# ansonb/RECON

Measured on AMD Instinct MI355X. Metric: edges aggregated/sec (GAT fwd+bwd) on synthetic KG-context graphs, higher is better.
Workload: dtype f32

## Files before the change

recon_amd/csrc/gat_atp.hip:

```cpp
#include <math.h>
#include <stdlib.h>
#include "recon_common.h"

#include <type_traits>

namespace recon {
namespace {

constexpr int kBlock = 256;

__device__ __forceinline__ int xcd_block(int b, int nb) {
    const int q = nb >> 3, r = nb & 7, x = b & 7, i = b >> 3;
    return (x < r ? x * (q + 1) : r * (q + 1) + (x - r) * q) + i;
}
template <int VEC, bool B16>
__device__ __forceinline__ void load_in(float (&r)[VEC], const float* base, int64_t e) {
    if constexpr (!B16) {
        load_vec<VEC>(r, base + e);
    } else {
        const uint16_t* b = reinterpret_cast<const uint16_t*>(base) + e;
        if constexpr (VEC == 4) {
            const uint2 t = *reinterpret_cast<const uint2*>(b);
            r[0] = __builtin_bit_cast(float, t.x << 16); r[1] = __builtin_bit_cast(float, t.x & 0xffff0000u);
            r[2] = __builtin_bit_cast(float, t.y << 16); r[3] = __builtin_bit_cast(float, t.y & 0xffff0000u);
// ... 1305 lines not shown
#endif
        if (hv && writer) {
            if (is_piece) p.hubG[static_cast<int64_t>(widx) * H + myh] = sum_gs;
            else p.Gs_dst[static_cast<int64_t>(node) * 2 * H + myh] = sum_gs;
        }
#pragma unroll
        for (int h = 0; h < HT; ++h) {
            if (h0 + h < H) {
                const float sh = lane_bcast(sum_gs, h << SH);
                const float* uh = U + (h0 + h) * UW;
#pragma unroll
                for (int r = 0; r < KR; ++r) {
                    float ud[VEC];
                    load_vec<VEC>(ud, uh + uF[r]);
#pragma unroll
                    for (int v = 0; v < VEC; ++v) gxd[r][v] = fmaf(sh, ud[v], gxd[r][v]);
                }
            }
        }
    }
    if (is_piece) return;
#ifdef RECON_K2_STAMPS
    stamp_[4] = __builtin_readcyclecounter();
    stamp_[5] = __builtin_amdgcn_s_getreg((31 << 11) | 4);
    if (lane == 0) {
        uint64_t* o = reinterpret_cast<uint64_t*>(p.gxd + static_cast<int64_t>(node) * F);
        for (int i = 0; i < 6; ++i) o[i] = stamp_[i];
        o[6] = static_cast<uint64_t>(end - beg);
    }
    if (!more) return;
    node = nnode; beg = nbeg; end = nend; srcv0 = nidx[0]; eidv0 = nidx[64];
    stamp_[0] = __builtin_readcyclecounter();
    continue;
#endif
    const auto rgx = K2_RSRC(p.gxd + static_cast<int64_t>(node) * F, F * 4);
#pragma unroll
    for (int r = 0; r < KR; ++r) buf_store_f32<VEC>(gxd[r], rgx, voF[r]);
    if (!more) return;
    node = nnode; beg = nbeg; end = nend; srcv0 = nidx[0]; eidv0 = nidx[64];
    }
}

template <int VEC>
__global__ void __launch_bounds__(kBlock) k_gat_atp_hub_bwd(const AtpBwdK p, const int32_t* __restrict__ hub_node, const int32_t* __restrict__ hub_ptr,
                                                            int32_t n_hub) {
    const int lane = threadIdx.x & 63;
    const int wave = __builtin_amdgcn_readfirstlane(threadIdx.x >> 6);
    const int t = blockIdx.x * (kBlock / 64) + wave;
    const int F = p.F, R = p.R, H = p.H, W = 2 * F + R;
    if (t >= n_hub) return;
    const int node = hub_node[t], p0 = hub_ptr[t], p1 = hub_ptr[t + 1];
    float tot = 0.f;
    if (lane < H) {
        float tt[1] = {0.f};
        sum_pieces<1>(tt, p.hubG + lane, H, p0, p1);
        tot = tt[0];
        p.Gs_dst[static_cast<int64_t>(node) * 2 * H + lane] += tot;
    }
    for (int c = lane * VEC; c < F; c += 64 * VEC) {
        float o[VEC];
        load_vec<VEC>(o, p.gxd + static_cast<int64_t>(node) * F + c);
        for (int h = 0; h < H; ++h) {
            const float sh = lane_bcast(tot, h);
            float ud[VEC];
            load_vec<VEC>(ud, p.u + static_cast<int64_t>(h) * W + c);
#pragma unroll
            for (int v = 0; v < VEC; ++v) o[v] = fmaf(sh, ud[v], o[v]);
        }
        store_vec<VEC>(p.gxd + static_cast<int64_t>(node) * F + c, o);
    }
}

struct AtpSrcK {
    const int32_t* rowptr_src; const int32_t* slot_by_src; const float* Gxs; const float* gxd; const float* gsigma;
    float* g_x; float* Gs_src;
    const float* u; int32_t W;
    int32_t N, F, H;
    int32_t hub_chunk, n_piece;
    const int4* piece;
    float* hubP;
    const int32_t* node_row;
};
template <int VEC, int KR>
__global__ void __launch_bounds__(kBlock) k_gat_atp_src(const AtpSrcK p) {
    const int lane = threadIdx.x & 63;
    const int wave = __builtin_amdgcn_readfirstlane(threadIdx.x >> 6);
    const int npb = (p.n_piece + kBlock / 64 - 1) / (kBlock / 64);
    const int widx = blockIdx.x * (kBlock / 64) + wave;
    const bool is_piece = static_cast<int>(blockIdx.x) < npb;
    int node = xcd_block(blockIdx.x - npb, gridDim.x - npb) * (kBlock / 64) + wave;
    int beg, end;
    if (is_piece) {
        if (widx >= p.n_piece) return;
        const int4 pc = p.piece[widx]; node = pc.x; beg = pc.y; end = pc.z;
    } else {
        if (node >= p.N) return;
        beg = p.rowptr_src[node]; end = p.rowptr_src[node + 1];
        if (p.hub_chunk && end - beg > p.hub_chunk) return;
    }
    const int F = p.F, H = p.H;
    const int drow = (p.node_row && !is_piece) ? p.node_row[node] : node;
    float acc[KR][VEC];
#pragma unroll
    for (int r = 0; r < KR; ++r) {
#pragma unroll
        for (int v = 0; v < VEC; ++v) acc[r][v] = 0.f;
        const int c = (r * 64 + lane) * VEC;
        if (!is_piece && c < F && p.g_x && drow >= 0) load_vec<VEC>(acc[r], p.gxd + static_cast<int64_t>(drow) * F + c);
    }
    float gs = 0.f;
    constexpr int U = 4;
    const int hl = lane < H ? lane : 0;
    for (int c0 = beg; c0 < end; c0 += 64) {
        const int cn = min(64, end - c0);
        const int slotv = p.slot_by_src[c0 + min(lane, cn - 1)];
        for (int j0 = 0; j0 < cn; j0 += U) {
            int slot[U];
#pragma unroll
            for (int u = 0; u < U; ++u) slot[u] = __builtin_amdgcn_readlane(slotv, min(j0 + u, cn - 1));
            float g4[U], t[U][KR][VEC];
#pragma unroll
            for (int u = 0; u < U; ++u) {
                g4[u] = p.gsigma[static_cast<int64_t>(slot[u]) * H + hl];
                if (p.g_x) {
#pragma unroll
                    for (int r = 0; r < KR; ++r) {
                        const int c = (r * 64 + lane) * VEC;
                        load_vec<VEC>(t[u][r], p.Gxs + static_cast<int64_t>(slot[u]) * F + (c < F ? c : 0));
                    }
                }
            }
#pragma unroll
            for (int u = 0; u < U; ++u) {
                if (j0 + u < cn) {
                    gs += g4[u];
                    if (p.g_x) {
#pragma unroll
                        for (int r = 0; r < KR; ++r)
#pragma unroll
                            for (int v = 0; v < VEC; ++v) acc[r][v] += t[u][r][v];
                    }
                }
            }
        }
    }
    float* gs_out = is_piece ? p.hubP + static_cast<int64_t>(widx) * (F + H) + F : p.Gs_src + static_cast<int64_t>(node) * 2 * H + H;
    float* row_out = is_piece ? p.hubP + static_cast<int64_t>(widx) * (F + H) : p.g_x + static_cast<int64_t>(node) * F;
    if (lane < H) gs_out[lane] = gs;
    if (!is_piece && p.g_x) {
        constexpr int HBK = KR <= 2 ? 8 : 2;
        for (int hb = 0; hb < H; hb += HBK) {
            float us[HBK][KR][VEC];
#pragma unroll
            for (int t = 0; t < HBK; ++t) {
                const float* uh = p.u + static_cast<int64_t>(min(hb + t, H - 1)) * p.W + F;
#pragma unroll
                for (int r = 0; r < KR; ++r) {
                    const int c = (r * 64 + lane) * VEC;
                    load_vec<VEC>(us[t][r], uh + (c < F ? c : 0));
                }
            }
#pragma unroll
            for (int t = 0; t < HBK; ++t) {
                const float sh = hb + t < H ? lane_bcast(gs, min(hb + t, 63)) : 0.f;
#pragma unroll
                for (int r = 0; r < KR; ++r)
#pragma unroll
                    for (int v = 0; v < VEC; ++v) acc[r][v] = fmaf(sh, us[t][r][v], acc[r][v]);
            }
        }
    }
    if (p.g_x) {
#pragma unroll
        for (int r = 0; r < KR; ++r) {
            const int c = (r * 64 + lane) * VEC;
            if (c < F) {
                if (is_piece && ((F + H) % VEC)) {
#pragma unroll
                    for (int v = 0; v < VEC; ++v) row_out[c + v] = acc[r][v];
                } else store_vec<VEC>(row_out + c, acc[r]);
            }
        }
    }
}

__global__ void __launch_bounds__(kBlock) k_gat_atp_hub_src(const AtpSrcK p, const int32_t* __restrict__ hub_node, const int32_t* __restrict__ hub_ptr,
                                                            int32_t n_hub) {
    const int lane = threadIdx.x & 63;
    const int F = p.F, H = p.H;
    const int stripes = (F + 63) / 64;
    const int idx = blockIdx.x * (kBlock / 64) + __builtin_amdgcn_readfirstlane(threadIdx.x >> 6);
    if (idx >= n_hub * stripes) return;
    const int t = idx / stripes, c = (idx - t * stripes) * 64 + lane;
    const int node = hub_node[t], p0 = hub_ptr[t], p1 = hub_ptr[t + 1];
    float gsl[1] = {0.f};
    if (lane < H) sum_pieces<1>(gsl, p.hubP + F + lane, F + H, p0, p1);
    if (c < H) p.Gs_src[static_cast<int64_t>(node) * 2 * H + H + c] = gsl[0];
    if (!p.g_x) return;
    const int drow = p.node_row ? p.node_row[node] : node;
    float a[1] = {(c < F && drow >= 0) ? p.gxd[static_cast<int64_t>(drow) * F + c] : 0.f};
    if (c < F) sum_pieces<1>(a, p.hubP + c, F + H, p0, p1);
    for (int h = 0; h < H; ++h) a[0] = fmaf(lane_bcast(gsl[0], h), p.u[static_cast<int64_t>(h) * p.W + F + (c < F ? c : 0)], a[0]);
    if (c < F) p.g_x[static_cast<int64_t>(node) * F + c] = a[0];
}


struct SkinnyJob { const float* G; const float* X; const int32_t* gather; float* partial; int32_t ldg, nj, rows, K, rpb, nb; };
template <int NJ, bool B16 = false>
__global__ void __launch_bounds__(256) k_skinny_tn_partial(const SkinnyJob j0, const SkinnyJob j1, const SkinnyJob j2) {
    __shared__ float red[3][NJ][256];
    const int which = static_cast<int>(blockIdx.x) < j0.nb ? 0 : (static_cast<int>(blockIdx.x) < j0.nb + j1.nb ? 1 : 2);
    const SkinnyJob& jb = which == 0 ? j0 : (which == 1 ? j1 : j2);
    const float* __restrict__ G = jb.G;
    const float* __restrict__ X = jb.X;
    const int32_t* __restrict__ gather = jb.gather;
    float* __restrict__ partial = jb.partial;
    const int ldg = jb.ldg, nj = jb.nj, rows = jb.rows, K = jb.K, rows_per_block = jb.rpb;
    const int bid = blockIdx.x - (which == 0 ? 0 : (which == 1 ? j0.nb : j0.nb + j1.nb));
    const int lane = threadIdx.x & 63, wave = threadIdx.x >> 6;
    const int r0 = bid * rows_per_block;
    const int r1 = min(rows, r0 + rows_per_block);
    for (int c0 = 0; c0 < K; c0 += 256) {
        const int c = c0 + 4 * lane;
        float acc[NJ][4];
#pragma unroll
        for (int j = 0; j < NJ; ++j) acc[j][0] = acc[j][1] = acc[j][2] = acc[j][3] = 0.f;
        int gi = 0;
        if (gather && lane < 4 && r0 + wave * 4 + lane < r1) gi = gather[r0 + wave * 4 + lane];
        for (int rb = r0 + wave * 4; rb < r1; rb += 16) {
            int gnext = 0;
            if (gather && lane < 4 && rb + 16 + lane < r1) gnext = gather[rb + 16 + lane];
            float xv[4][4];
            float gl = 0.f;
            {
                const int q = lane / NJ, j = lane % NJ;
                if (q < 4 && rb + q < r1 && j < nj) gl = G[static_cast<int64_t>(rb + q) * ldg + j];
            }
#pragma unroll
            for (int q = 0; q < 4; ++q) {
                const int r = rb + q;
                xv[q][0] = xv[q][1] = xv[q][2] = xv[q][3] = 0.f;
                if (r < r1) {
                    const int64_t row = gather ? __builtin_amdgcn_readlane(gi, q) : r;
                    if constexpr (B16) {
                        if (c + 3 < K) load_in<4, true>(xv[q], X, row * K + c);
                    } else {
                        if (c + 3 < K) { const float4 t = *reinterpret_cast<const float4*>(X + row * K + c); xv[q][0] = t.x; xv[q][1] = t.y; xv[q][2] = t.z; xv[q][3] = t.w; }
                        else { for (int v = 0; v < 4; ++v) if (c + v < K) xv[q][v] = X[row * K + c + v]; }
                    }
                }
            }
            gi = gnext;
            float gv[4][NJ];
#pragma unroll
            for (int q = 0; q < 4; ++q)
#pragma unroll
                for (int j = 0; j < NJ; ++j) gv[q][j] = (q * NJ + j < 64) ? lane_bcast(gl, (q * NJ + j) & 63) : 0.f;
#pragma unroll
            for (int q = 0; q < 4; ++q)
#pragma unroll
                for (int j = 0; j < NJ; ++j)
#pragma unroll
                    for (int v = 0; v < 4; ++v) acc[j][v] = fmaf(gv[q][j], xv[q][v], acc[j][v]);
        }
        __syncthreads();
        if (wave > 0) {
#pragma unroll
            for (int j = 0; j < NJ; ++j)
#pragma unroll
                for (int v = 0; v < 4; ++v) red[wave - 1][j][4 * lane + v] = acc[j][v];
        }
        __syncthreads();
        if (wave == 0) {
#pragma unroll
            for (int j = 0; j < NJ; ++j)
                if (j < nj)
#pragma unroll
                    for (int v = 0; v < 4; ++v)
                        if (c + v < K)
                            partial[(static_cast<int64_t>(bid) * nj + j) * K + c + v] =
                                ((acc[j][v] + red[0][j][4 * lane + v]) + red[1][j][4 * lane + v]) + red[2][j][4 * lane + v];
        }
    }
}
struct SkinnyRedJob { const float* partial; float* out; int64_t S1, S2; int32_t nb, nj, K, P, nblocks; };
__global__ void __launch_bounds__(1024) k_skinny_reduce(const SkinnyRedJob j0, const SkinnyRedJob j1, const SkinnyRedJob j2) {
    __shared__ float red[64][17];
    const int which = static_cast<int>(blockIdx.x) < j0.nblocks ? 0 : (static_cast<int>(blockIdx.x) < j0.nblocks + j1.nblocks ? 1 : 2);
    const SkinnyRedJob& jb = which == 0 ? j0 : (which == 1 ? j1 : j2);
    const float* __restrict__ partial = jb.partial;
    float* __restrict__ out = jb.out;
    const int nb = jb.nb, nj = jb.nj, K = jb.K, P = jb.P;
    const int64_t S1 = jb.S1, S2 = jb.S2;
    const int bid = blockIdx.x - (which == 0 ? 0 : (which == 1 ? j0.nblocks : j0.nblocks + j1.nblocks));
    const int e = threadIdx.x & 15, grp = threadIdx.x >> 4;
    const int idx = bid * 16 + e;
    const int tot = nj * K;
    const int per = (nb + 63) / 64;
    const int b0 = grp * per, b1 = min(nb, (grp + 1) * per);
    float s0 = 0.f, s1 = 0.f, s2 = 0.f, s3 = 0.f;
    if (idx < tot) {
        int b = b0;
        for (; b + 4 <= b1; b += 4) {
            s0 += partial[static_cast<int64_t>(b) * tot + idx];
            s1 += partial[static_cast<int64_t>(b + 1) * tot + idx];
            s2 += partial[static_cast<int64_t>(b + 2) * tot + idx];
            s3 += partial[static_cast<int64_t>(b + 3) * tot + idx];
        }
        for (; b < b1; ++b) s0 += partial[static_cast<int64_t>(b) * tot + idx];
    }
    red[grp][e] = (s0 + s1) + (s2 + s3);
    __syncthreads();
    if (grp == 0 && idx < tot) {
        float t = 0.f;
#pragma unroll
        for (int g = 0; g < 64; ++g) t += red[g][e];
        const int j = idx / K, c = idx % K;
        out[(j % P) * S1 + (j / P) * S2 + c] = t;
    }
}

struct AtpShape { int vec, kr, ht; };
bool atp_shape(int F, int R, int H, AtpShape* s) {
    const int mx = F > R ? F : R;
    int vec;
    if (F % 4 == 0 && R % 4 == 0) vec = 4;
    else if (F % 2 == 0 && R % 2 == 0) vec = 2;
    else return false;
    int kr = (mx + 64 * vec - 1) / (64 * vec);
    if (kr > 2 && kr <= 4) kr = 4; else if (kr > 4 && kr <= 8) kr = 8; else if (kr > 8) return false;
    int ht = 1;
    while (ht < H && ht < 8) ht <<= 1;
    while (ht > 1 && 2 * ht * kr * vec > 96) ht >>= 1;
    if (2 * ht * kr * vec > 96) return false;
    s->vec = vec; s->kr = kr; s->ht = ht;
    return true;
}
bool al(const void* p, size_t a) { return (reinterpret_cast<uintptr_t>(p) & (a - 1)) == 0; }
int atp_key(const AtpShape& s) { return s.vec * 1000 + s.kr * 10 + (s.ht == 8 ? 3 : s.ht == 4 ? 2 : s.ht == 2 ? 1 : 0); }

#define ATP_DISPATCH(S, CALL)                                                                              \
    do {                                                                                                   \
        const int key_ = atp_key(S);                                                                       \
        switch (key_) {                                                                                    \
            case 4010: CALL(4, 1, 1); break; case 4011: CALL(4, 1, 2); break; case 4012: CALL(4, 1, 4); break; case 4013: CALL(4, 1, 8); break; \
            case 4020: CALL(4, 2, 1); break; case 4021: CALL(4, 2, 2); break; case 4022: CALL(4, 2, 4); break;   \
            case 4040: CALL(4, 4, 1); break; case 4041: CALL(4, 4, 2); break; case 4080: CALL(4, 8, 1); break;   \
            case 2010: CALL(2, 1, 1); break; case 2011: CALL(2, 1, 2); break; case 2012: CALL(2, 1, 4); break; case 2013: CALL(2, 1, 8); break; \
            case 2020: CALL(2, 2, 1); break; case 2021: CALL(2, 2, 2); break; case 2022: CALL(2, 2, 4); break; case 2023: CALL(2, 2, 8); break; \
            case 2040: CALL(2, 4, 1); break; case 2041: CALL(2, 4, 2); break; case 2042: CALL(2, 4, 4); break;   \
            case 2080: CALL(2, 8, 1); break; case 2081: CALL(2, 8, 2); break;                                   \
            default: return RECON_ERR_UNSUPPORTED;                                                         \
        }                                                                                                  \
    } while (0)

int check_atp(const recon_graph* g, const recon_gat_atp_args* a) {
    if (!g || !a) return RECON_ERR_INVALID;
    if (a->N != g->N || a->E != g->E) return RECON_ERR_INVALID;
    if (a->N < 0 || a->E < 0 || a->F <= 0 || a->R <= 0 || a->D <= 0 || a->H <= 0) return RECON_ERR_INVALID;
    if (a->ld_out < a->H * a->D) return RECON_ERR_INVALID;
    if (!a->x || !a->a || !a->a_2 || !a->u || !a->c_node || !a->V || !a->out) return RECON_ERR_INVALID;
    if (a->E > 0 && (!a->edge_embed || !a->c_rel)) return RECON_ERR_INVALID;
    if (a->H > 4096) return RECON_ERR_UNSUPPORTED;
    if (a->ee_index && a->E > 0 && a->ee_rows <= 0) return RECON_ERR_INVALID;
    return RECON_OK;
}

// ... 211 lines not shown

extern "C" int recon_gat_atp_project(const recon_graph* g, const recon_gat_atp_args* a, recon_stream_t stream) {
    AtpShape s;
    int rc = atp_fwd_common(g, a, &s);
    if (rc != RECON_OK) return rc;
    if (a->N == 0) return RECON_OK;
    const int32_t W = 2 * a->F + a->R;
    const int32_t NR = atp_rows(g, a).n;
    OperandDesc A = plain_operand(a->V, static_cast<int64_t>(a->H) * W);
    OperandDesc B = plain_operand(a->a, W);
    OutputDesc C = plain_output(a->out, a->ld_out);
    GemmBatch bt;
    bt.batch = a->H; bt.a_bs = W; bt.b_bs = static_cast<int64_t>(a->D) * W; bt.c_bs = a->D;
    bt.epilogue = a->concat ? 1 : 0;
    if (atp_hx2(a))
        return gemm_hx2_batched(NR, a->D, W, a->V, W, 2LL * W, 2LL * NR * W, a->a_split, C, bt, atp_scale_v(a), atp_scale_a(a),
                                as_stream(stream), atp_dst_shared(a));
    if (a->a_split && bx3_supported(A, W, bt)) return gemm_bx3_batched(NR, a->D, W, A, a->a_split, C, bt, as_stream(stream));
    return gemm_f32_batched(NR, a->D, W, A, true, B, true, C, bt, 1, nullptr, as_stream(stream));
}

namespace {
__global__ void __launch_bounds__(kBlock) k_rows_expand(const float* __restrict__ rows, int32_t ld_rows, const int32_t* __restrict__ node_row, int32_t N,
                                                        int32_t width, float* __restrict__ out, int32_t ld_out, int32_t vec4) {
    const int lane = threadIdx.x & 63;
    const int n = blockIdx.x * (kBlock / 64) + __builtin_amdgcn_readfirstlane(threadIdx.x >> 6);
    if (n >= N) return;
    const int r = node_row[n];
    float* o = out + static_cast<int64_t>(n) * ld_out;
    const float* in = rows + static_cast<int64_t>(r < 0 ? 0 : r) * ld_rows;
    if (vec4) {
        for (int c = 4 * lane; c < width; c += 256) {
            const float4 v = r >= 0 ? *reinterpret_cast<const float4*>(in + c) : make_float4(0.f, 0.f, 0.f, 0.f);
            *reinterpret_cast<float4*>(o + c) = v;
        }
    } else {
        for (int c = lane; c < width; c += 64) o[c] = r >= 0 ? in[c] : 0.f;
    }
}
}
extern "C" int recon_rows_expand(const float* rows, int32_t ld_rows, const int32_t* node_row, int32_t N, int32_t width, float* out, int32_t ld_out,
                                 recon_stream_t stream) {
    if (N < 0 || width < 0 || ld_rows < width || ld_out < width || (N > 0 && (!node_row || !out)) || (N > 0 && width > 0 && !rows)) return RECON_ERR_INVALID;
    if (N == 0 || width == 0) return RECON_OK;
    const int vec4 = ((width | ld_rows | ld_out) & 3) == 0 && !((reinterpret_cast<uintptr_t>(rows) | reinterpret_cast<uintptr_t>(out)) & 15);
    hipLaunchKernelGGL(k_rows_expand, dim3(static_cast<unsigned>(ceil_div64(N, kBlock / 64))), dim3(kBlock), 0, as_stream(stream), rows, ld_rows, node_row, N, width, out,
                       ld_out, vec4);
    RECON_CHECK_LAUNCH();
    return RECON_OK;
}

extern "C" int recon_gat_atp_fwd(const recon_graph* g, const recon_gat_atp_args* a, recon_stream_t stream) {
    int rc = recon_gat_atp_scores(g, a, stream);
    if (rc != RECON_OK) return rc;
    rc = recon_gat_atp_aggregate(g, a, stream);
    if (rc != RECON_OK) return rc;
    return recon_gat_atp_project(g, a, stream);
}

extern "C" int recon_gat_atp_bwd_gee_bf16_supported(int32_t F, int32_t R, int32_t D, int32_t H) {
    recon::AtpShape s;
    if (!recon_gat_atp_bf16_io_supported(F, R, D, H) || !recon::atp_shape(F, R, H, &s)) return 0;
    const size_t lds_k2 = static_cast<size_t>(H) * (F + R) * sizeof(float) + (kBlock / 64) * 512;
    const bool lring = s.vec == 4 && s.kr == 1 && lds_k2 + (kBlock / 64) * kK2LdsRingBytes <= 64 * 1024 && cfg_char(CFG_K2_LDS_RING) != '0';
    return (s.ht >= H && lring) ? 1 : 0;
}

extern "C" size_t recon_gat_atp_bwd_split_bytes(int32_t N, int32_t D, int32_t H) {
    if (N <= 0 || D <= 0 || H <= 0) return 256;
    return align_up(static_cast<size_t>(3) * N * bx3_kp(H * D) * 2, 256);
}

extern "C" size_t recon_gat_atp_bwd_partial_floats(int32_t N, int32_t E, int32_t F, int32_t R, int32_t D, int32_t H) {
    const int64_t W = 2LL * F + R;
    int s1 = gemm_pick_split_k(static_cast<int32_t>(W), D, N, H);
    const int s2 = bx3_kmajor_splits(N, bx3_kmajor_split_k(static_cast<int32_t>(W), D, N, H));
    if (s2 > s1) s1 = s2;
    size_t need = static_cast<size_t>(s1) * H * D * W;
    (void)E; (void)F; (void)R;
    return need > 0 ? need : 1;
}

constexpr int kSkinnySlices = 1024;
extern "C" size_t recon_gat_atp_bwd_partial2_floats(int32_t N, int32_t E, int32_t F, int32_t R, int32_t D, int32_t H) {
    (void)N; (void)E; (void)D; (void)H;
    const size_t mx = static_cast<size_t>(F > R ? F : R);
    return static_cast<size_t>(3) * kSkinnySlices * 16 * mx;
}

extern "C" int recon_gat_atp_bwd(const recon_graph* g, const recon_gat_atp_bwd_args* b, recon_stream_t stream) {
    return recon_gat_atp_bwd_phase(g, b, RECON_ATP_BWD_ALL, stream);
}

extern "C" int recon_gat_atp_bwd_phase(const recon_graph* g, const recon_gat_atp_bwd_args* b, int32_t phases, recon_stream_t stream) {
    if (!b) return RECON_ERR_INVALID;
    const recon_gat_atp_args* a = &b->fwd;
    int rc = check_atp(g, a);
    if (rc != RECON_OK) return rc;
    if (!recon_gat_atp_supported(a->N, a->E, a->F, a->R, a->D, a->H)) return RECON_ERR_UNSUPPORTED;
    if (!a->Z || !a->Zk || !b->grad_out || !b->g_V || !b->gxd || !b->Gs || !b->g_u || !b->partial || !b->partial2 || !b->q) return RECON_ERR_INVALID;
    if (a->E > 0 && (!a->sigma || !b->g_sigma || !b->Gxs)) return RECON_ERR_INVALID;
    const bool hx2 = atp_hx2(a);
    if ((a->concat || atp_rows(g, a).row_node) && !b->g_h && !hx2) return RECON_ERR_INVALID;
    if (hx2 && (!b->gh_split || (reinterpret_cast<uintptr_t>(b->gh_split) & 15) || (b->ld_gout & 3))) return RECON_ERR_INVALID;
    if (b->ld_gout < a->H * a->D) return RECON_ERR_INVALID;
    if (a->N == 0) return RECON_OK;
    hipStream_t st = as_stream(stream);
    const int32_t N = a->N, E = a->E, F = a->F, R = a->R, D = a->D, H = a->H, W = 2 * F + R;
    const AtpRows rw = atp_rows(g, a);
    const int32_t NR = rw.n;
    const int64_t HD = 1LL * H * D;
    AtpShape s;
    atp_shape(F, R, H, &s);
    const size_t lds_u = static_cast<size_t>(H) * (F + R) * sizeof(float);
    if (lds_u > 60 * 1024) return RECON_ERR_UNSUPPORTED;
    const size_t lds_k2 = lds_u + (kBlock / 64) * 512;

    const float* gh = b->grad_out;
    int32_t ld_gh = b->ld_gout;
    const int64_t ld_ghp = bx3_kp(static_cast<int32_t>(HD));
    const bool gh_planes = hx2 || (b->gh_split && a->a_split && !(reinterpret_cast<uintptr_t>(b->gh_split) & 15) && (D % 8) == 0 &&
                                   ((b->ld_gout | a->ld_out) & 3) == 0);
    uint16_t* ghp = gh_planes ? static_cast<uint16_t*>(b->gh_split) : nullptr;
    const int64_t ldi = (static_cast<int64_t>(NR) + 7) / 8 * 8;
    const size_t inv_off = align_up(static_cast<size_t>(2) * N * bx3_kp(static_cast<int32_t>(HD)) * 2, 256);
    const bool row_scaled = hx2 && D <= 256 && ((a->ld_out | b->ld_gout) & 3) == 0 && cfg_char(CFG_ATP_ROW_SCALE) != '0' &&
                            inv_off + static_cast<size_t>(H) * ldi * sizeof(float) <= recon_gat_atp_bwd_split_bytes(N, D, H);
    float* row_inv = row_scaled ? reinterpret_cast<float*>(static_cast<char*>(b->gh_split) + inv_off) : nullptr;
    if (phases & RECON_ATP_BWD_PREPARE) {
        if (hx2 && !row_scaled) {
            rc = hx2_amax(b->grad_out, N, static_cast<int32_t>(HD), b->ld_gout, atp_q(a, 3), st);
            if (rc != RECON_OK) return rc;
        }
        hipLaunchKernelGGL(k_elu_grad_q, dim3(static_cast<unsigned>(ceil_div64(1LL * NR * H, 16))), dim3(256), 0, st, b->grad_out, b->ld_gout, a->out,
                           a->ld_out, NR, H, D, a->concat, ((a->concat || rw.row_node) && !hx2) ? b->g_h : nullptr, b->q, ghp, hx2 ? 2LL * D : ld_ghp,
                           hx2 ? static_cast<int64_t>(D) : static_cast<int64_t>(NR) * ld_ghp, hx2 ? 1 : 0,
                           hx2 ? atp_scale_g(a) : Hx2Scale{nullptr, nullptr, 1.f}, row_inv, ldi, row_scaled ? atp_q(a, 3) : nullptr, rw.row_node);
    }
    if (a->concat || rw.row_node) { gh = b->g_h; ld_gh = static_cast<int32_t>(HD); }
    GemmBatch bt;
    bt.batch = H; bt.epilogue = 0;
    if (phases & RECON_ATP_BWD_INPUTS) {
    {
        OperandDesc A = plain_operand(gh, ld_gh);
        OperandDesc B = plain_operand(a->a, W);
        OutputDesc C = plain_output(b->g_V, static_cast<int64_t>(H) * W);
        bt.a_bs = D; bt.b_bs = static_cast<int64_t>(D) * W; bt.c_bs = W;
        if (hx2)
            rc = gemm_hx2_batched(NR, W, D, b->gh_split, D, 2LL * D, 2LL * NR * D,
                                  static_cast<const char*>(a->a_split) + split_part_bytes(D, W, H), C, bt,
                                  row_scaled ? Hx2Scale{nullptr, nullptr, 1.f} : atp_scale_g(a), atp_scale_a(a), st, 0, row_inv, ldi);
        else if (a->a_split && bx3_supported(A, D, bt))
            rc = gemm_bx3_batched(NR, W, D, A, static_cast<const char*>(a->a_split) + split_part_bytes(D, W, H), C, bt, st);
        else
            rc = gemm_f32_batched(NR, W, D, A, true, B, false, C, bt, 1, nullptr, st);
        if (rc != RECON_OK) return rc;
    }
    {
        AtpBwdK p;
        p.rowptr = rw.rowptr; p.row_node = rw.row_node; p.src = g->src; p.eid = a->ee_index ? a->ee_index : g->eid;
        p.gee_by_slot = a->ee_index ? 1 : 0;
        p.gee_b16 = b->g_ee_bf16 ? 1 : 0;
        if (b->g_ee_bf16 && !(a->io_bf16 && !a->ee_index && b->g_edge_embed && recon_gat_atp_bwd_gee_bf16_supported(F, R, D, H))) return RECON_ERR_UNSUPPORTED;
        p.x = a->x; p.ee = a->edge_embed; p.keep = a->keep; p.sigma = a->sigma; p.Z = a->Z; p.Zk = a->Zk;
        p.q = b->q; p.gV = b->g_V; p.u = a->u;
        p.gsigma = b->g_sigma; p.Gs_dst = b->Gs; p.Gxs = b->Gxs; p.gxd = b->gxd; p.g_ee = b->g_edge_embed;
        p.N = NR; p.E = E; p.F = F; p.R = R; p.H = H; p.alpha = a->alpha;
        const bool hubs = atp_hubs(g);
        if (hubs && static_cast<size_t>(g->hub_ws_floats) < recon_graph_hub_ws_floats(g, F, R, H)) return RECON_ERR_WORKSPACE;
        p.hub_chunk = hubs ? g->hub_chunk : 0; p.n_piece = hubs ? g->n_piece : 0;
        p.piece = reinterpret_cast<const int4*>(g->piece); p.hubG = g->hub_ws;
        dim3 grid;
        const bool lring = s.vec == 4 && s.kr == 1 && lds_k2 + (kBlock / 64) * kK2LdsRingBytes <= 64 * 1024 && cfg_char(CFG_K2_LDS_RING) != '0';
        const size_t lds_run = lds_k2 + (lring ? (kBlock / 64) * kK2LdsRingBytes : 0);
#define CALL_BWD(V_, K_, H_) do { constexpr bool LRC = V_ == 4 && K_ == 1;                                                                   \
                                  if (V_ == 4 && a->io_bf16) { if (LRC && lring && p.gee_b16) hipLaunchKernelGGL((k_gat_atp_bwd<4, K_, H_, true, LRC, LRC>), grid, dim3(kBlock), lds_run, st, p); \
                                                               else if (LRC && lring) hipLaunchKernelGGL((k_gat_atp_bwd<4, K_, H_, true, LRC>), grid, dim3(kBlock), lds_run, st, p); \
                                                               else hipLaunchKernelGGL((k_gat_atp_bwd<4, K_, H_, true>), grid, dim3(kBlock), lds_run, st, p); }          \
                                  else if (LRC && lring) hipLaunchKernelGGL((k_gat_atp_bwd<V_, K_, H_, false, LRC>), grid, dim3(kBlock), lds_run, st, p);              \
                                  else hipLaunchKernelGGL((k_gat_atp_bwd<V_, K_, H_>), grid, dim3(kBlock), lds_run, st, p); } while (0)
        p.persist = (p.n_piece == 0 && cfg_char(CFG_K2_PERSIST) != '0') ? 1 : 0;
        if (p.persist) {
            const int64_t need = ceil_div64(NR, kBlock / 64);
            int64_t nb = k2_resident_blocks(s.kr, s.ht, lds_run);
            if (nb > need) nb = (need + 7) / 8 * 8;
            grid = dim3(static_cast<unsigned>(nb));
        } else {
            grid = dim3(static_cast<unsigned>(ceil_div64(NR, kBlock / 64) + ceil_div64(p.n_piece, kBlock / 64)));
        }
        ATP_DISPATCH(s, CALL_BWD);
#undef CALL_BWD
        if (hubs) {
            const dim3 gh(static_cast<unsigned>(ceil_div64(g->n_hub, kBlock / 64)));
            if (s.vec == 4) hipLaunchKernelGGL((k_gat_atp_hub_bwd<4>), gh, dim3(kBlock), 0, st, p, g->hub_node, g->hub_ptr, g->n_hub);
            else hipLaunchKernelGGL((k_gat_atp_hub_bwd<2>), gh, dim3(kBlock), 0, st, p, g->hub_node, g->hub_ptr, g->n_hub);
        }
        RECON_CHECK_LAUNCH();
    }
    {
        AtpSrcK p;
        p.rowptr_src = g->rowptr_src; p.slot_by_src = g->slot_by_src; p.Gxs = b->Gxs; p.gxd = b->gxd; p.gsigma = b->g_sigma;
        p.g_x = b->g_x; p.Gs_src = b->Gs; p.u = a->u; p.W = W;
        p.N = N; p.F = F; p.H = H; p.node_row = rw.node_row;
        const bool hubs = g->hub_chunk > 0 && g->n_hub_src > 0 && g->n_piece_src > 0 && g->hub_node_src && g->hub_ptr_src && g->piece_src && g->hub_ws;
        if (hubs && static_cast<size_t>(g->hub_ws_floats) < recon_graph_hub_ws_floats(g, F, R, H)) return RECON_ERR_WORKSPACE;
        p.hub_chunk = hubs ? g->hub_chunk : 0; p.n_piece = hubs ? g->n_piece_src : 0;
        p.piece = reinterpret_cast<const int4*>(g->piece_src); p.hubP = g->hub_ws;
        dim3 grid(static_cast<unsigned>(ceil_div64(N, kBlock / 64) + ceil_div64(p.n_piece, kBlock / 64)));
        const int key = s.vec * 10 + s.kr;
        switch (key) {
            case 41: hipLaunchKernelGGL((k_gat_atp_src<4, 1>), grid, dim3(kBlock), 0, st, p); break;
            case 42: hipLaunchKernelGGL((k_gat_atp_src<4, 2>), grid, dim3(kBlock), 0, st, p); break;
            case 44: hipLaunchKernelGGL((k_gat_atp_src<4, 4>), grid, dim3(kBlock), 0, st, p); break;
            case 48: hipLaunchKernelGGL((k_gat_atp_src<4, 8>), grid, dim3(kBlock), 0, st, p); break;
            case 21: hipLaunchKernelGGL((k_gat_atp_src<2, 1>), grid, dim3(kBlock), 0, st, p); break;
            case 22: hipLaunchKernelGGL((k_gat_atp_src<2, 2>), grid, dim3(kBlock), 0, st, p); break;
            case 24: hipLaunchKernelGGL((k_gat_atp_src<2, 4>), grid, dim3(kBlock), 0, st, p); break;
            default: hipLaunchKernelGGL((k_gat_atp_src<2, 8>), grid, dim3(kBlock), 0, st, p); break;
        }
        if (hubs) hipLaunchKernelGGL(k_gat_atp_hub_src, dim3(static_cast<unsigned>(ceil_div64(1LL * g->n_hub_src * ceil_div64(F, 64), kBlock / 64))), dim3(kBlock), 0, st, p,
                                     g->hub_node_src, g->hub_ptr_src, g->n_hub_src);
        RECON_CHECK_LAUNCH();
    }
    }
    if (b->g_a || b->g_a_2) {
        if (!b->g_a) return RECON_ERR_INVALID;
        if (phases & RECON_ATP_BWD_WEIGHTS) {
            OperandDesc A = plain_operand(a->V, static_cast<int64_t>(H) * W);
            OperandDesc B = plain_operand(gh, ld_gh);
            OutputDesc C = plain_output(b->g_a, W);
            GemmBatch bw = bt;
            bw.a_bs = W; bw.b_bs = D; bw.c_bs = static_cast<int64_t>(D) * W; bw.c_transpose = 1;
            const int64_t ldv = static_cast<int64_t>(H) * W;
            if (hx2) {
                const int sk = bx3_kmajor_splits(NR, bx3_kmajor_split_k(W, D, NR, H));
                rc = gemm_hx2_kmajor_batched(W, D, NR, a->V, 2LL * W, W, 2LL * NR * W, b->gh_split, 2LL * D, D, 2LL * NR * D,
                                             H, sk, b->partial, static_cast<const char*>(a->aux) + kHx2ZeroPageOffset, atp_scale_v(a), atp_scale_g(a), st,
                                             atp_dst_shared(a), row_inv, ldi);
                if (rc == RECON_OK && (phases & RECON_ATP_BWD_EARLY_SUM)) rc = splitk_reduce(b->partial, sk, W, D, C, bw.c_bs, H, 0, true, st);
            } else if (gh_planes && bx3_kmajor_supported(a->V, ldv, W, ld_ghp, D, W, D)) {
                const int sk = bx3_kmajor_splits(NR, bx3_kmajor_split_k(W, D, NR, H));
                rc = gemm_bx3_kmajor_batched(W, D, NR, a->V, ldv, W, b->gh_split, ld_ghp, static_cast<int64_t>(NR) * ld_ghp, D, H, sk, b->partial, st);
                if (rc == RECON_OK) rc = splitk_reduce(b->partial, sk, W, D, C, bw.c_bs, H, 0, true, st);
            } else {
                const int sk = gemm_pick_split_k(W, D, NR, H);
                rc = gemm_f32_batched(W, D, NR, A, false, B, false, C, bw, sk, b->partial, st);
            }
            if (rc != RECON_OK) return rc;
        }
        if (phases & RECON_ATP_BWD_INPUTS) {
            struct Prod { const float* G; int ldg, nj; const float* X; const int32_t* gather; int rows, K, P; int64_t S1, S2; float* out; };
            const int32_t* ee_gather = a->ee_index ? a->ee_index : g->eid;
            const size_t third = recon_gat_atp_bwd_partial2_floats(N, E, F, R, D, H) / 3;
            auto run_jobs = [&](const Prod* pr, int count) {
                SkinnyJob sj[3];
                SkinnyRedJob rj[3];
                int nj_max = 0, nb_total = 0, nr_total = 0;
                for (int i = 0; i < 3; ++i) {
                    sj[i] = SkinnyJob{nullptr, nullptr, nullptr, nullptr, 0, 0, 0, 0, 1, 0};
                    rj[i] = SkinnyRedJob{nullptr, nullptr, 0, 0, 0, 0, 0, 1, 0};
                    if (i >= count) continue;
                    const Prod& q = pr[i];
                    if (q.rows <= 0) {
                        for (int j = 0; j < q.nj; ++j) (void)hipMemsetAsync(q.out + (j % q.P) * q.S1 + (j / q.P) * q.S2, 0, sizeof(float) * q.K, st);
                        continue;
                    }
                    int rpb = static_cast<int>(ceil_div64(q.rows, kSkinnySlices));
                    if (rpb < 32) rpb = 32;
                    const int nb = static_cast<int>(ceil_div64(q.rows, rpb));
                    float* part = b->partial2 + i * third;
                    sj[i] = SkinnyJob{q.G, q.X, q.gather, part, q.ldg, q.nj, q.rows, q.K, rpb, nb};
                    rj[i] = SkinnyRedJob{part, q.out, q.S1, q.S2, nb, q.nj, q.K, q.P, static_cast<int32_t>(ceil_div64(1LL * q.nj * q.K, 16))};
                    if (q.nj > nj_max) nj_max = q.nj;
                    nb_total += nb; nr_total += rj[i].nblocks;
                }
                if (nb_total == 0) return;
                const dim3 gp(static_cast<unsigned>(nb_total));
                if (a->io_bf16) {
                    if (nj_max <= 8) hipLaunchKernelGGL((k_skinny_tn_partial<8, true>), gp, dim3(256), 0, st, sj[0], sj[1], sj[2]);
                    else hipLaunchKernelGGL((k_skinny_tn_partial<16, true>), gp, dim3(256), 0, st, sj[0], sj[1], sj[2]);
                } else if (nj_max <= 8) hipLaunchKernelGGL((k_skinny_tn_partial<8>), gp, dim3(256), 0, st, sj[0], sj[1], sj[2]);
                else hipLaunchKernelGGL((k_skinny_tn_partial<16>), gp, dim3(256), 0, st, sj[0], sj[1], sj[2]);
                hipLaunchKernelGGL(k_skinny_reduce, dim3(static_cast<unsigned>(nr_total)), dim3(1024), 0, st, rj[0], rj[1], rj[2]);
            };
            if (H <= 8) {
                const Prod pr[3] = {{b->Gs, 2 * H, H, a->x, rw.row_node, NR, F, H, W, 0, b->g_u},
                                    {b->Gs + H, 2 * H, H, a->x, nullptr, N, F, H, W, 0, b->g_u + F},
                                    {b->g_sigma, H, H, a->edge_embed, ee_gather, E, R, H, W, 0, b->g_u + 2 * F}};
                run_jobs(pr, 3);
            } else {
                for (int j = 0; j < 2 * H; ++j) {
                    const Prod one = {b->Gs + j, 2 * H, 1, a->x, j < H ? rw.row_node : nullptr, j < H ? NR : N, F, 1, W, 0,
                                      b->g_u + static_cast<int64_t>(j % H) * W + (j / H) * F};
                    run_jobs(&one, 1);
                }
                for (int h0 = 0; h0 < H; h0 += 16) {
                    const int nh = H - h0 < 16 ? H - h0 : 16;
                    const Prod one = {b->g_sigma + h0, H, nh, a->edge_embed, ee_gather, E, R, nh, W, 0, b->g_u + static_cast<int64_t>(h0) * W + 2 * F};
                    run_jobs(&one, 1);
                }
            }
            RECON_CHECK_LAUNCH();
        }
        if ((phases & RECON_ATP_BWD_FINISH) && hx2 && !(phases & RECON_ATP_BWD_EARLY_SUM)) {
            const int sk = bx3_kmajor_splits(NR, bx3_kmajor_split_k(W, D, NR, H));
            const int ntile = static_cast<int>(ceil_div64(W, 32) * ceil_div64(D, 32)) * H;
            hipLaunchKernelGGL(k_atp_weights_finish, dim3(static_cast<unsigned>(ntile + ceil_div64(1LL * H * D, 8))), dim3(256), 0, st, b->partial, sk, W,
                               D, H, a->a, a->a_2, b->g_u, b->g_a, b->g_a_2, atp_q(a, 3), kHx2QuantityWords);
        } else if (phases & RECON_ATP_BWD_FINISH)
        hipLaunchKernelGGL(k_score_vec_bwd, dim3(static_cast<unsigned>(D), static_cast<unsigned>(H)), dim3(256), 0, st, a->a, a->a_2, b->g_u,
                           D, W, b->g_a, b->g_a_2, atp_hx2(a) ? atp_q(a, 3) : nullptr, kHx2QuantityWords);
        RECON_CHECK_LAUNCH();
    } else if ((phases & RECON_ATP_BWD_FINISH) && atp_hx2(a)) {
        if (hipMemsetAsync(atp_q(a, 3), 0, sizeof(uint32_t) * kHx2QuantityWords, st) != hipSuccess) return RECON_ERR_LAUNCH;
    }
    return RECON_OK;
}
```

Measured before the change: 80.92 million.

## Fuse source-gradient kernel with skinny weight-gradient partials in one launch

Merges the per-source-node gradient kernel and the skinny TN weight-gradient partial kernel into a single grid. The first blocks run the source-side wave work and the rest run skinny partial tiles. For the source job, the skinny blocks recompute per-row summed g_sigma from the CSR into LDS instead of reading the Gs source half from global memory, which removes a dependency and lets both kernels overlap. It also cuts the shared reduction buffer from three slices to one, reducing sequentially wave by wave. That lowers LDS use at the cost of extra barriers. The weight-gradient launch moves from the later phase block into the source phase, which may change phase semantics.

```diff
diff --git a/recon_amd/csrc/gat_atp.hip b/recon_amd/csrc/gat_atp.hip
--- a/recon_amd/csrc/gat_atp.hip
+++ b/recon_amd/csrc/gat_atp.hip
@@ -1411,13 +1411,13 @@
     const int32_t* node_row;
 };
 template <int VEC, int KR>
-__global__ void __launch_bounds__(kBlock) k_gat_atp_src(const AtpSrcK p) {
+__device__ __forceinline__ void atp_src_wave(const AtpSrcK& p, int bx, int nbx) {
     const int lane = threadIdx.x & 63;
     const int wave = __builtin_amdgcn_readfirstlane(threadIdx.x >> 6);
     const int npb = (p.n_piece + kBlock / 64 - 1) / (kBlock / 64);
-    const int widx = blockIdx.x * (kBlock / 64) + wave;
-    const bool is_piece = static_cast<int>(blockIdx.x) < npb;
-    int node = xcd_block(blockIdx.x - npb, gridDim.x - npb) * (kBlock / 64) + wave;
+    const int widx = bx * (kBlock / 64) + wave;
+    const bool is_piece = bx < npb;
+    int node = xcd_block(bx - npb, nbx - npb) * (kBlock / 64) + wave;
     int beg, end;
     if (is_piece) {
         if (widx >= p.n_piece) return;
@@ -1512,6 +1512,9 @@
         }
     }
 }
+
+template <int VEC, int KR>
+__global__ void __launch_bounds__(kBlock) k_gat_atp_src(const AtpSrcK p) { atp_src_wave<VEC, KR>(p, blockIdx.x, gridDim.x); }
 
 __global__ void __launch_bounds__(kBlock) k_gat_atp_hub_src(const AtpSrcK p, const int32_t* __restrict__ hub_node, const int32_t* __restrict__ hub_ptr,
                                                             int32_t n_hub) {
@@ -1535,38 +1538,53 @@
 
 
 struct SkinnyJob { const float* G; const float* X; const int32_t* gather; float* partial; int32_t ldg, nj, rows, K, rpb, nb; };
-template <int NJ, bool B16 = false>
-__global__ void __launch_bounds__(256) k_skinny_tn_partial(const SkinnyJob j0, const SkinnyJob j1, const SkinnyJob j2) {
-    __shared__ float red[3][NJ][256];
-    const int which = static_cast<int>(blockIdx.x) < j0.nb ? 0 : (static_cast<int>(blockIdx.x) < j0.nb + j1.nb ? 1 : 2);
-    const SkinnyJob& jb = which == 0 ? j0 : (which == 1 ? j1 : j2);
+struct SkinnySrc { const int32_t* rowptr_src; const int32_t* slot_by_src; const float* gsigma; };
+template <int NJ, bool B16, bool SRC>
+__device__ __forceinline__ void skinny_block(const SkinnyJob& jb, int bid, float (&red)[NJ][256], float* __restrict__ gsl, const SkinnySrc& sr, bool src) {
+    constexpr int RPI = 4;
     const float* __restrict__ G = jb.G;
     const float* __restrict__ X = jb.X;
     const int32_t* __restrict__ gather = jb.gather;
     float* __restrict__ partial = jb.partial;
     const int ldg = jb.ldg, nj = jb.nj, rows = jb.rows, K = jb.K, rows_per_block = jb.rpb;
-    const int bid = blockIdx.x - (which == 0 ? 0 : (which == 1 ? j0.nb : j0.nb + j1.nb));
     const int lane = threadIdx.x & 63, wave = threadIdx.x >> 6;
     const int r0 = bid * rows_per_block;
     const int r1 = min(rows, r0 + rows_per_block);
+    if (SRC && src) {
+        const int n = (r1 - r0) * nj;
+        for (int i = threadIdx.x; i < n; i += 256) {
+            const int rr = i / nj, h = i - rr * nj;
+            const int beg = sr.rowptr_src[r0 + rr], end = sr.rowptr_src[r0 + rr + 1];
+            float gs = 0.f;
+            for (int c0 = beg; c0 < end; c0 += 4) {
+                float g4[4];
+#pragma unroll
+                for (int u = 0; u < 4; ++u) g4[u] = sr.gsigma[static_cast<int64_t>(sr.slot_by_src[min(c0 + u, end - 1)]) * nj + h];
+#pragma unroll
+                for (int u = 0; u < 4; ++u) if (c0 + u < end) gs += g4[u];
+            }
+            gsl[i] = gs;
+        }
+        __syncthreads();
+    }
     for (int c0 = 0; c0 < K; c0 += 256) {
         const int c = c0 + 4 * lane;
         float acc[NJ][4];
 #pragma unroll
         for (int j = 0; j < NJ; ++j) acc[j][0] = acc[j][1] = acc[j][2] = acc[j][3] = 0.f;
         int gi = 0;
-        if (gather && lane < 4 && r0 + wave * 4 + lane < r1) gi = gather[r0 + wave * 4 + lane];
-        for (int rb = r0 + wave * 4; rb < r1; rb += 16) {
+        if (gather && lane < RPI && r0 + wave * RPI + lane < r1) gi = gather[r0 + wave * RPI + lane];
+        for (int rb = r0 + wave * RPI; rb < r1; rb += 4 * RPI) {
             int gnext = 0;
-            if (gather && lane < 4 && rb + 16 + lane < r1) gnext = gather[rb + 16 + lane];
-            float xv[4][4];
+            if (gather && lane < RPI && rb + 4 * RPI + lane < r1) gnext = gather[rb + 4 * RPI + lane];
+            float xv[RPI][4];
             float gl = 0.f;
             {
                 const int q = lane / NJ, j = lane % NJ;
-                if (q < 4 && rb + q < r1 && j < nj) gl = G[static_cast<int64_t>(rb + q) * ldg + j];
-            }
-#pragma unroll
-            for (int q = 0; q < 4; ++q) {
+                if (q < RPI && rb + q < r1 && j < nj) gl = (SRC && src) ? gsl[(rb + q - r0) * nj + j] : G[static_cast<int64_t>(rb + q) * ldg + j];
+            }
+#pragma unroll
+            for (int q = 0; q < RPI; ++q) {
                 const int r = rb + q;
                 xv[q][0] = xv[q][1] = xv[q][2] = xv[q][3] = 0.f;
                 if (r < r1) {
@@ -1580,38 +1598,63 @@
                 }
             }
             gi = gnext;
-            float gv[4][NJ];
-#pragma unroll
-            for (int q = 0; q < 4; ++q)
-#pragma unroll
-                for (int j = 0; j < NJ; ++j) gv[q][j] = (q * NJ + j < 64) ? lane_bcast(gl, (q * NJ + j) & 63) : 0.f;
-#pragma unroll
-            for (int q = 0; q < 4; ++q)
+#pragma unroll
+            for (int q = 0; q < RPI; ++q)
+#pragma unroll
+                for (int j = 0; j < NJ; ++j) {
+                    const float gv = lane_bcast(gl, q * NJ + j);
+#pragma unroll
+                    for (int v = 0; v < 4; ++v) acc[j][v] = fmaf(gv, xv[q][v], acc[j][v]);
+                }
+        }
+        for (int w = 1; w < 4; ++w) {
+            __syncthreads();
+            if (wave == w) {
 #pragma unroll
                 for (int j = 0; j < NJ; ++j)
 #pragma unroll
-                    for (int v = 0; v < 4; ++v) acc[j][v] = fmaf(gv[q][j], xv[q][v], acc[j][v]);
-        }
-        __syncthreads();
-        if (wave > 0) {
-#pragma unroll
-            for (int j = 0; j < NJ; ++j)
-#pragma unroll
-                for (int v = 0; v < 4; ++v) red[wave - 1][j][4 * lane + v] = acc[j][v];
-        }
-        __syncthreads();
+                    for (int v = 0; v < 4; ++v) red[j][4 * lane + v] = acc[j][v];
+            }
+            __syncthreads();
+            if (wave == 0) {
+#pragma unroll
+                for (int j = 0; j < NJ; ++j)
+#pragma unroll
+                    for (int v = 0; v < 4; ++v) acc[j][v] += red[j][4 * lane + v];
+            }
+        }
         if (wave == 0) {
 #pragma unroll
             for (int j = 0; j < NJ; ++j)
                 if (j < nj)
 #pragma unroll
                     for (int v = 0; v < 4; ++v)
-                        if (c + v < K)
-                            partial[(static_cast<int64_t>(bid) * nj + j) * K + c + v] =
-                                ((acc[j][v] + red[0][j][4 * lane + v]) + red[1][j][4 * lane + v]) + red[2][j][4 * lane + v];
-        }
-    }
-}
+                        if (c + v < K) partial[(static_cast<int64_t>(bid) * nj + j) * K + c + v] = acc[j][v];
+        }
+    }
+}
+template <int NJ, bool B16 = false>
+__global__ void __launch_bounds__(256) k_skinny_tn_partial(const SkinnyJob j0, const SkinnyJob j1, const SkinnyJob j2) {
+    __shared__ float red[NJ][256];
+    const int which = static_cast<int>(blockIdx.x) < j0.nb ? 0 : (static_cast<int>(blockIdx.x) < j0.nb + j1.nb ? 1 : 2);
+    const SkinnyJob& jb = which == 0 ? j0 : (which == 1 ? j1 : j2);
+    skinny_block<NJ, B16, false>(jb, blockIdx.x - (which == 0 ? 0 : (which == 1 ? j0.nb : j0.nb + j1.nb)), red, nullptr, SkinnySrc{nullptr, nullptr, nullptr}, false);
+}
+
+template <int VEC, int KR, bool B16>
+__global__ void __launch_bounds__(kBlock) k_gat_atp_src_skinny(const AtpSrcK p, int32_t nsrc, const SkinnyJob j0, const SkinnyJob j1, const SkinnyJob j2,
+                                                               const SkinnySrc sr) {
+    static_assert(kBlock == 256, "skinny_block: 4 waves");
+    __shared__ float red[8][256];
+    extern __shared__ __attribute__((aligned(16))) float gsl[];
+    const int bx = blockIdx.x;
+    if (bx < nsrc) { atp_src_wave<VEC, KR>(p, bx, nsrc); return; }
+    const int b = bx - nsrc;
+    const int which = b < j0.nb ? 0 : (b < j0.nb + j1.nb ? 1 : 2);
+    const SkinnyJob& jb = which == 0 ? j0 : (which == 1 ? j1 : j2);
+    skinny_block<8, B16, true>(jb, b - (which == 0 ? 0 : (which == 1 ? j0.nb : j0.nb + j1.nb)), red, gsl, sr, which == 1);
+}
+
 struct SkinnyRedJob { const float* partial; float* out; int64_t S1, S2; int32_t nb, nj, K, P, nblocks; };
 __global__ void __launch_bounds__(1024) k_skinny_reduce(const SkinnyRedJob j0, const SkinnyRedJob j1, const SkinnyRedJob j2) {
     __shared__ float red[64][17];
@@ -1989,6 +2032,11 @@
 }
 
 constexpr int kSkinnySlices = 1024;
+constexpr size_t kSkinnySrcLdsMax = 32 * 1024;
+static int skinny_rpb(int64_t rows) {
+    const int rpb = static_cast<int>(ceil_div64(rows, kSkinnySlices));
+    return rpb < 32 ? 32 : rpb;
+}
 extern "C" size_t recon_gat_atp_bwd_partial2_floats(int32_t N, int32_t E, int32_t F, int32_t R, int32_t D, int32_t H) {
     (void)N; (void)E; (void)D; (void)H;
     const size_t mx = static_cast<size_t>(F > R ? F : R);
@@ -2113,20 +2161,84 @@
         if (hubs && static_cast<size_t>(g->hub_ws_floats) < recon_graph_hub_ws_floats(g, F, R, H)) return RECON_ERR_WORKSPACE;
         p.hub_chunk = hubs ? g->hub_chunk : 0; p.n_piece = hubs ? g->n_piece_src : 0;
         p.piece = reinterpret_cast<const int4*>(g->piece_src); p.hubP = g->hub_ws;
-        dim3 grid(static_cast<unsigned>(ceil_div64(N, kBlock / 64) + ceil_div64(p.n_piece, kBlock / 64)));
-        const int key = s.vec * 10 + s.kr;
-        switch (key) {
-            case 41: hipLaunchKernelGGL((k_gat_atp_src<4, 1>), grid, dim3(kBlock), 0, st, p); break;
-            case 42: hipLaunchKernelGGL((k_gat_atp_src<4, 2>), grid, dim3(kBlock), 0, st, p); break;
-            case 44: hipLaunchKernelGGL((k_gat_atp_src<4, 4>), grid, dim3(kBlock), 0, st, p); break;
-            case 48: hipLaunchKernelGGL((k_gat_atp_src<4, 8>), grid, dim3(kBlock), 0, st, p); break;
-            case 21: hipLaunchKernelGGL((k_gat_atp_src<2, 1>), grid, dim3(kBlock), 0, st, p); break;
-            case 22: hipLaunchKernelGGL((k_gat_atp_src<2, 2>), grid, dim3(kBlock), 0, st, p); break;
-            case 24: hipLaunchKernelGGL((k_gat_atp_src<2, 4>), grid, dim3(kBlock), 0, st, p); break;
-            default: hipLaunchKernelGGL((k_gat_atp_src<2, 8>), grid, dim3(kBlock), 0, st, p); break;
-        }
-        if (hubs) hipLaunchKernelGGL(k_gat_atp_hub_src, dim3(static_cast<unsigned>(ceil_div64(1LL * g->n_hub_src * ceil_div64(F, 64), kBlock / 64))), dim3(kBlock), 0, st, p,
-                                     g->hub_node_src, g->hub_ptr_src, g->n_hub_src);
+        const bool want_u = b->g_a || b->g_a_2;
+        if (want_u && !b->g_a) return RECON_ERR_INVALID;
+        const size_t lds_src = static_cast<size_t>(skinny_rpb(N)) * H * sizeof(float);
+        const bool share = want_u && H <= 8 && !hubs && lds_src <= kSkinnySrcLdsMax && (!a->io_bf16 || s.vec == 4);
+        const int nsrc = static_cast<int>(ceil_div64(N, kBlock / 64) + ceil_div64(p.n_piece, kBlock / 64));
+        SkinnyJob sj[3];
+        int nb_total = 0;
+        auto launch_src = [&]() -> int {
+            const dim3 grid(static_cast<unsigned>(nsrc + (share ? nb_total : 0)));
+            const SkinnySrc sr{g->rowptr_src, g->slot_by_src, b->g_sigma};
+#define CALL_SRC(V_, K_) do { if (!share) hipLaunchKernelGGL((k_gat_atp_src<V_, K_>), grid, dim3(kBlock), 0, st, p);                                          \
+                              else if (V_ == 4 && a->io_bf16) hipLaunchKernelGGL((k_gat_atp_src_skinny<4, K_, true>), grid, dim3(kBlock), lds_src, st, p, nsrc, sj[0], sj[1], sj[2], sr); \
+                              else hipLaunchKernelGGL((k_gat_atp_src_skinny<V_, K_, false>), grid, dim3(kBlock), lds_src, st, p, nsrc, sj[0], sj[1], sj[2], sr); } while (0)
+            switch (s.vec * 10 + s.kr) {
+                case 41: CALL_SRC(4, 1); break; case 42: CALL_SRC(4, 2); break; case 44: CALL_SRC(4, 4); break; case 48: CALL_SRC(4, 8); break;
+                case 21: CALL_SRC(2, 1); break; case 22: CALL_SRC(2, 2); break; case 24: CALL_SRC(2, 4); break; default: CALL_SRC(2, 8); break;
+            }
+#undef CALL_SRC
+            if (hubs) hipLaunchKernelGGL(k_gat_atp_hub_src, dim3(static_cast<unsigned>(ceil_div64(1LL * g->n_hub_src * ceil_div64(F, 64), kBlock / 64))), dim3(kBlock), 0, st, p,
+                                         g->hub_node_src, g->hub_ptr_src, g->n_hub_src);
+            return RECON_OK;
+        };
+        if (!share) launch_src();
+        if (want_u) {
+            struct Prod { const float* G; int ldg, nj; const float* X; const int32_t* gather; int rows, K, P; int64_t S1, S2; float* out; };
+            const int32_t* ee_gather = a->ee_index ? a->ee_index : g->eid;
+            const size_t third = recon_gat_atp_bwd_partial2_floats(N, E, F, R, D, H) / 3;
+            auto run_jobs = [&](const Prod* pr, int count) {
+                SkinnyRedJob rj[3];
+                int nj_max = 0, nr_total = 0;
+                nb_total = 0;
+                for (int i = 0; i < 3; ++i) {
+                    sj[i] = SkinnyJob{nullptr, nullptr, nullptr, nullptr, 0, 0, 0, 0, 1, 0};
+                    rj[i] = SkinnyRedJob{nullptr, nullptr, 0, 0, 0, 0, 0, 1, 0};
+                    if (i >= count) continue;
+                    const Prod& q = pr[i];
+                    if (q.rows <= 0) {
+                        for (int j = 0; j < q.nj; ++j) (void)hipMemsetAsync(q.out + (j % q.P) * q.S1 + (j / q.P) * q.S2, 0, sizeof(float) * q.K, st);
+                        continue;
+                    }
+                    const int rpb = skinny_rpb(q.rows);
+                    const int nb = static_cast<int>(ceil_div64(q.rows, rpb));
+                    float* part = b->partial2 + i * third;
+                    sj[i] = SkinnyJob{q.G, q.X, q.gather, part, q.ldg, q.nj, q.rows, q.K, rpb, nb};
+                    rj[i] = SkinnyRedJob{part, q.out, q.S1, q.S2, nb, q.nj, q.K, q.P, static_cast<int32_t>(ceil_div64(1LL * q.nj * q.K, 16))};
+                    if (q.nj > nj_max) nj_max = q.nj;
+                    nb_total += nb; nr_total += rj[i].nblocks;
+                }
+                if (share) { launch_src(); if (nb_total == 0) return; }
+                else {
+                    if (nb_total == 0) return;
+                    const dim3 gp(static_cast<unsigned>(nb_total));
+                    if (a->io_bf16) {
+                        if (nj_max <= 8) hipLaunchKernelGGL((k_skinny_tn_partial<8, true>), gp, dim3(256), 0, st, sj[0], sj[1], sj[2]);
+                        else hipLaunchKernelGGL((k_skinny_tn_partial<16, true>), gp, dim3(256), 0, st, sj[0], sj[1], sj[2]);
+                    } else if (nj_max <= 8) hipLaunchKernelGGL((k_skinny_tn_partial<8>), gp, dim3(256), 0, st, sj[0], sj[1], sj[2]);
+                    else hipLaunchKernelGGL((k_skinny_tn_partial<16>), gp, dim3(256), 0, st, sj[0], sj[1], sj[2]);
+                }
+                hipLaunchKernelGGL(k_skinny_reduce, dim3(static_cast<unsigned>(nr_total)), dim3(1024), 0, st, rj[0], rj[1], rj[2]);
+            };
+            if (H <= 8) {
+                const Prod pr[3] = {{b->Gs, 2 * H, H, a->x, rw.row_node, NR, F, H, W, 0, b->g_u},
+                                    {b->Gs + H, 2 * H, H, a->x, nullptr, N, F, H, W, 0, b->g_u + F},
+                                    {b->g_sigma, H, H, a->edge_embed, ee_gather, E, R, H, W, 0, b->g_u + 2 * F}};
+                run_jobs(pr, 3);
+            } else {
+                for (int j = 0; j < 2 * H; ++j) {
+                    const Prod one = {b->Gs + j, 2 * H, 1, a->x, j < H ? rw.row_node : nullptr, j < H ? NR : N, F, 1, W, 0,
+                                      b->g_u + static_cast<int64_t>(j % H) * W + (j / H) * F};
+                    run_jobs(&one, 1);
+                }
+                for (int h0 = 0; h0 < H; h0 += 16) {
+                    const int nh = H - h0 < 16 ? H - h0 : 16;
+                    const Prod one = {b->g_sigma + h0, H, nh, a->edge_embed, ee_gather, E, R, nh, W, 0, b->g_u + static_cast<int64_t>(h0) * W + 2 * F};
+                    run_jobs(&one, 1);
+                }
+            }
+        }
         RECON_CHECK_LAUNCH();
     }
     }
@@ -2155,60 +2267,6 @@
             }
             if (rc != RECON_OK) return rc;
         }
-        if (phases & RECON_ATP_BWD_INPUTS) {
-            struct Prod { const float* G; int ldg, nj; const float* X; const int32_t* gather; int rows, K, P; int64_t S1, S2; float* out; };
-            const int32_t* ee_gather = a->ee_index ? a->ee_index : g->eid;
-            const size_t third = recon_gat_atp_bwd_partial2_floats(N, E, F, R, D, H) / 3;
-            auto run_jobs = [&](const Prod* pr, int count) {
-                SkinnyJob sj[3];
-                SkinnyRedJob rj[3];
-                int nj_max = 0, nb_total = 0, nr_total = 0;
-                for (int i = 0; i < 3; ++i) {
-                    sj[i] = SkinnyJob{nullptr, nullptr, nullptr, nullptr, 0, 0, 0, 0, 1, 0};
-                    rj[i] = SkinnyRedJob{nullptr, nullptr, 0, 0, 0, 0, 0, 1, 0};
-                    if (i >= count) continue;
-                    const Prod& q = pr[i];
-                    if (q.rows <= 0) {
-                        for (int j = 0; j < q.nj; ++j) (void)hipMemsetAsync(q.out + (j % q.P) * q.S1 + (j / q.P) * q.S2, 0, sizeof(float) * q.K, st);
-                        continue;
-                    }
-                    int rpb = static_cast<int>(ceil_div64(q.rows, kSkinnySlices));
-                    if (rpb < 32) rpb = 32;
-                    const int nb = static_cast<int>(ceil_div64(q.rows, rpb));
-                    float* part = b->partial2 + i * third;
-                    sj[i] = SkinnyJob{q.G, q.X, q.gather, part, q.ldg, q.nj, q.rows, q.K, rpb, nb};
-                    rj[i] = SkinnyRedJob{part, q.out, q.S1, q.S2, nb, q.nj, q.K, q.P, static_cast<int32_t>(ceil_div64(1LL * q.nj * q.K, 16))};
-                    if (q.nj > nj_max) nj_max = q.nj;
-                    nb_total += nb; nr_total += rj[i].nblocks;
-                }
-                if (nb_total == 0) return;
-                const dim3 gp(static_cast<unsigned>(nb_total));
-                if (a->io_bf16) {
-                    if (nj_max <= 8) hipLaunchKernelGGL((k_skinny_tn_partial<8, true>), gp, dim3(256), 0, st, sj[0], sj[1], sj[2]);
-                    else hipLaunchKernelGGL((k_skinny_tn_partial<16, true>), gp, dim3(256), 0, st, sj[0], sj[1], sj[2]);
-                } else if (nj_max <= 8) hipLaunchKernelGGL((k_skinny_tn_partial<8>), gp, dim3(256), 0, st, sj[0], sj[1], sj[2]);
-                else hipLaunchKernelGGL((k_skinny_tn_partial<16>), gp, dim3(256), 0, st, sj[0], sj[1], sj[2]);
-                hipLaunchKernelGGL(k_skinny_reduce, dim3(static_cast<unsigned>(nr_total)), dim3(1024), 0, st, rj[0], rj[1], rj[2]);
-            };
-            if (H <= 8) {
-                const Prod pr[3] = {{b->Gs, 2 * H, H, a->x, rw.row_node, NR, F, H, W, 0, b->g_u},
-                                    {b->Gs + H, 2 * H, H, a->x, nullptr, N, F, H, W, 0, b->g_u + F},
-                                    {b->g_sigma, H, H, a->edge_embed, ee_gather, E, R, H, W, 0, b->g_u + 2 * F}};
-                run_jobs(pr, 3);
-            } else {
-                for (int j = 0; j < 2 * H; ++j) {
-                    const Prod one = {b->Gs + j, 2 * H, 1, a->x, j < H ? rw.row_node : nullptr, j < H ? NR : N, F, 1, W, 0,
-                                      b->g_u + static_cast<int64_t>(j % H) * W + (j / H) * F};
-                    run_jobs(&one, 1);
-                }
-                for (int h0 = 0; h0 < H; h0 += 16) {
-                    const int nh = H - h0 < 16 ? H - h0 : 16;
-                    const Prod one = {b->g_sigma + h0, H, nh, a->edge_embed, ee_gather, E, R, nh, W, 0, b->g_u + static_cast<int64_t>(h0) * W + 2 * F};
-                    run_jobs(&one, 1);
-                }
-            }
-            RECON_CHECK_LAUNCH();
-        }
         if ((phases & RECON_ATP_BWD_FINISH) && hx2 && !(phases & RECON_ATP_BWD_EARLY_SUM)) {
             const int sk = bx3_kmajor_splits(NR, bx3_kmajor_split_k(W, D, NR, H));
             const int ntile = static_cast<int>(ceil_div64(W, 32) * ceil_div64(D, 32)) * H;
```

Result: faster. 82.40 million, median of 6 (+1.8%).
